# maltezfaria/LevelSetMethods.jl

Hardware: AMD Instinct MI355X
Metric: Mcells/s per RK3 step (WENO5 advect+reinit), 512^3 fp64; HBM GB/s vs peak (higher is better)
Workload: dtype f64; 1 GPU; 3D 512^3 vortex-deformation WENO5 advection + EikonalReinitializationTerm, RK3, NeumannBC, fp64; cells=134217728, integrator=RK3, arithmetic_mode=fast, parallelism=single, halo_overlap=n/a, prewarm_steps=10, exchange=n/a

## Files before the change

levelsetmethods.jl_amd/csrc/stage_brick.h:

```cpp
#pragma once
#include "stage_kernel.h"

namespace lsm {
namespace LSM_NS {

template <class LT>
struct LdsElems {
    const LT* p;
    LSM_DEV double operator[](int i) const { return (double)p[i]; }
};
template <int W, int HW, class LT>
struct BrickView {
    LdsElems<LT> T0;
    double c;
    LSM_DEV double z(int k) const { return T0[k * HW]; }
    template <int D>
    LSM_DEV double at(int k) const { return T0[k * (D == 0 ? 1 : (D == 1 ? W : HW))]; }
    template <int A, int B>
    LSM_DEV double corner(int sa, int sb) const { return T0[sa * (A == 0 ? 1 : W) + sb * (B == 1 ? W : HW)]; }
};

#ifndef LSM_BRICK_PITCH
#define LSM_BRICK_PITCH 44
#endif
struct BrickCfg {
    static constexpr int TX = 32, TY = 8, XL = 4;
    static constexpr int W = TX + 2 * XL;
    static constexpr int WP = LSM_BRICK_PITCH;
    static_assert(WP >= W && WP % 4 == 0, "rows hold the loaded elements and start on 16-byte boundaries");
};

template <int ADV, int NM, int CURV, int EIK, class ST, int AK, int NT, int BZ>
__global__ void __launch_bounds__(NT) brick_kernel(const StageArgs a, const unsigned sub_per) {
    constexpr int NDIM = 3, TX = BrickCfg::TX, TY = BrickCfg::TY, XL = BrickCfg::XL, W = BrickCfg::W, WP = BrickCfg::WP;
    constexpr int G = halo_of(ADV, NM, CURV, EIK);
    constexpr int SEG = 16 / (int)sizeof(ST), NSEG = W / SEG, PSEG = WP / SEG;
    constexpr int H = TY + 2 * G, HW = H * WP, D = BZ + 2 * G;
    constexpr int NROW = D * H, NV4 = NROW * PSEG;
    constexpr int BPT = TX * TY * BZ / NT;
    static_assert(XL >= G && XL % SEG == 0 && W % SEG == 0 && (BPT == 8 || BPT == 4) && NT % 64 == 0, "");
    __shared__ lsm_v4u vbrick[NV4];
    __shared__ unsigned short nodes[TX * TY * BZ];
    __shared__ int wsum[NT / 64];
    static_assert(2 * (sizeof(lsm_v4u) * NV4 + sizeof(unsigned short) * TX * TY * BZ + 64) <= 160 * 1024, "brick kernel: LDS budget of a gfx950 CU");
    const ST* brick = reinterpret_cast<const ST*>(vbrick);

    const unsigned nwg = a.nbrick_list * sub_per, per = (nwg + 7u) / 8u;
    const unsigned wg = (blockIdx.x % 8u) * per + blockIdx.x / 8u;
    if (blockIdx.x / 8u >= per || wg >= nwg) return;
    const unsigned tile_id = (unsigned)a.brick_list[wg / sub_per], sub = wg % sub_per;
    const unsigned tbx = tile_id % a.nb[0], tby = (tile_id / a.nb[0]) % a.nb[1], tbm = tile_id / (a.nb[0] * a.nb[1]);
    const int bx0 = tbx * TX, by0 = tby * TY;
    const int nx = a.n[0], ny = a.n[1], nm = a.n[2];
    const long long sy = a.s1, sm = a.s2;
    const int m0 = a.mb + (int)tbm * a.mc;
    const int m1 = m0 + a.mc < a.me ? m0 + a.mc : a.me;
    const int zb = m0 + (int)sub * BZ;
    if (zb >= m1) return;
    const int nz = m1 - zb < BZ ? m1 - zb : BZ;
    const int tid = threadIdx.x, lane = tid & 63, wv = tid >> 6;
    unsigned long long mbytes;
    const int mrow = tid / (TX / BPT), mq = tid % (TX / BPT), mzr = mrow / TY, myr = mrow % TY;
    {
        const unsigned char* mb_ = uniform_ptr(a.mask + (a.origin + (long long)zb * sm + (long long)by0 * sy + bx0));
        const bool rv = mzr < nz && by0 + myr < ny;
        const unsigned moff = rv ? (unsigned)mzr * (unsigned)sm + (unsigned)myr * (unsigned)sy + (unsigned)(mq * BPT) : LSM_OOB_OFFSET;
        if constexpr (BPT == 8) mbytes = __builtin_bit_cast(unsigned long long, __builtin_amdgcn_raw_buffer_load_b64(plane_rsrc(mb_), moff, 0, 0));
        else mbytes = __builtin_amdgcn_raw_buffer_load_b32(plane_rsrc(mb_), moff, 0, 0);
    }
    constexpr int RPI = NT / NSEG, NIT = (NROW + RPI - 1) / RPI, QZ = RPI / H, RY = RPI % H;
    lsm_v4u v[NIT];
    const int crow = tid / NSEG, cseg = tid - crow * NSEG;
    {
        const ST* cb = uniform_ptr(reinterpret_cast<const ST*>(a.psi) + (a.origin + (long long)(zb - G) * sm + (long long)(by0 - G) * sy + (bx0 - XL)));
        const bool cv = crow < RPI && bx0 - XL + cseg * SEG <= nx + G - 1;
        int zr = crow / H, yr = crow - zr * H;
#pragma unroll
        for (int k = 0; k < NIT; ++k) {
            int Y = by0 - G + yr, Z = zb - G + zr;
            Y = Y > ny + G - 1 ? ny + G - 1 : Y;
            Z = Z > nm + G - 1 ? nm + G - 1 : Z;
            const unsigned eo = (unsigned)(Z - (zb - G)) * (unsigned)sm + (unsigned)(Y - (by0 - G)) * (unsigned)sy + (unsigned)(cseg * SEG);
            const unsigned off = (cv && zr < D) ? (unsigned)sizeof(ST) * eo : LSM_OOB_OFFSET;
            v[k] = __builtin_bit_cast(lsm_v4u, __builtin_amdgcn_raw_buffer_load_b128(plane_rsrc(cb), off, 0, 0));
            yr += RY; zr += QZ;
            if (yr >= H) { yr -= H; ++zr; }
        }
    }
    int N;
    {
        unsigned bits = 0;
#pragma unroll
        for (int j = 0; j < BPT; ++j)
            if (((mbytes >> (8 * j)) & 0xffull) != 0 && bx0 + mq * BPT + j < nx) bits |= 1u << j;
        const int cnt = __builtin_popcount(bits);
// ... 95 lines not shown
```

levelsetmethods.jl_amd/csrc/stage_kernel.h:

```cpp
#pragma once
#include <cstdlib>
#include <type_traits>
#include "lsm_internal.h"
#include "stage_math.h"

namespace lsm {
namespace LSM_NS {

#if LSM_STRICT
constexpr bool ADV_SCALED = false;
#else
constexpr bool ADV_SCALED = true;
#endif
constexpr int adv_factor_kind(int ADV, bool PLAIN) {
#if LSM_STRICT
    return 0;
#else
    return ADV == 2 ? (LSM_T1 ? 1 : 0) | (LSM_T2 && PLAIN ? 2 : 0) : 0;
#endif
}
template <int FK>
LSM_DEV double adv_factor(const StageArgs& a, int k) {
    if constexpr (FK == 3) return a.cdt_inv_h3[k];
    else if constexpr (FK == 2) return a.cdt * a.inv_h[k];
    else if constexpr (FK == 1) return a.inv_h3[k];
    else return a.inv_h[k];
}

constexpr int halo_of(int ADV, int NM, int CURV, int EIK) {
    int g = 0;
    if (ADV == 2) g = 3;
    if (ADV == 1 && g < 1) g = 1;
    if ((NM || EIK) && g < 2) g = 2;
    if (CURV && g < 1) g = 1;
    return g;
}

template <class T>
LSM_DEV T* uniform_ptr(T* p) {
    const unsigned long long v = reinterpret_cast<unsigned long long>(p);
    const unsigned lo = __builtin_amdgcn_readfirstlane((unsigned)v), hi = __builtin_amdgcn_readfirstlane((unsigned)(v >> 32));
    return reinterpret_cast<T*>(((unsigned long long)hi << 32) | lo);
}
LSM_DEV double ld_uniform(const double* t, int i) {
    typedef const __attribute__((address_space(4))) double* cptr;
    return *((cptr)(unsigned long long)t + i);
}
typedef unsigned lsm_v2u __attribute__((ext_vector_type(2)));
LSM_DEV __amdgpu_buffer_rsrc_t plane_rsrc(const void* base, int range = (int)0x80000000u) {
    return __builtin_amdgcn_make_buffer_rsrc(const_cast<void*>(base), 0, range, 0x00020000);
}
constexpr unsigned LSM_OOB_OFFSET = 0xC0000000u;
template <class ST, int AUX = 0>
LSM_DEV double ldg(const ST* base, unsigned boff, int range = (int)0x80000000u) {
    if constexpr (sizeof(ST) == 8) return __builtin_bit_cast(double, __builtin_amdgcn_raw_buffer_load_b64(plane_rsrc(base, range), boff, 0, AUX));
    else return (double)__builtin_bit_cast(float, __builtin_amdgcn_raw_buffer_load_b32(plane_rsrc(base, range), boff, 0, AUX));
}
template <class ST, int AUX = 0>
LSM_DEV void stg(ST* base, unsigned boff, double v) {
    if constexpr (sizeof(ST) == 8) __builtin_amdgcn_raw_buffer_store_b64(__builtin_bit_cast(lsm_v2u, v), plane_rsrc(base), boff, 0, AUX);
    else __builtin_amdgcn_raw_buffer_store_b32(__builtin_bit_cast(unsigned, (float)v), plane_rsrc(base), boff, 0, AUX);
}
typedef unsigned lsm_v4u __attribute__((ext_vector_type(4)));
template <class ST, int AUX = 0>
LSM_DEV void ldg2(const ST* base, unsigned boff, double& x, double& y, int range = (int)0x80000000u) {
    if constexpr (sizeof(ST) == 8) {
        const lsm_v4u v = __builtin_bit_cast(lsm_v4u, __builtin_amdgcn_raw_buffer_load_b128(plane_rsrc(base, range), boff, 0, AUX));
        x = __builtin_bit_cast(double, lsm_v2u{v.x, v.y});
        y = __builtin_bit_cast(double, lsm_v2u{v.z, v.w});
    } else {
        const unsigned long long u = __builtin_bit_cast(unsigned long long, __builtin_amdgcn_raw_buffer_load_b64(plane_rsrc(base, range), boff, 0, AUX));
        x = (double)__builtin_bit_cast(float, (unsigned)u);
        y = (double)__builtin_bit_cast(float, (unsigned)(u >> 32));
    }
}
template <class ST, int AUX = 0>
LSM_DEV void stg2(ST* base, unsigned boff, double x, double y) {
    if constexpr (sizeof(ST) == 8) {
        const lsm_v2u a = __builtin_bit_cast(lsm_v2u, x), b = __builtin_bit_cast(lsm_v2u, y);
        __builtin_amdgcn_raw_buffer_store_b128(lsm_v4u{a.x, a.y, b.x, b.y}, plane_rsrc(base), boff, 0, AUX);
    } else {
        const unsigned long long u = (unsigned long long)__builtin_bit_cast(unsigned, (float)x) | ((unsigned long long)__builtin_bit_cast(unsigned, (float)y) << 32);
        __builtin_amdgcn_raw_buffer_store_b64(__builtin_bit_cast(lsm_v2u, u), plane_rsrc(base), boff, 0, AUX);
    }
}
LSM_DEV unsigned ldg_u8(const unsigned char* base, unsigned boff, int range) {
    return __builtin_amdgcn_raw_buffer_load_b8(
        __builtin_amdgcn_make_buffer_rsrc(const_cast<unsigned char*>(base), 0, __builtin_amdgcn_readfirstlane(range), 0x00020000), boff, 0, 0);
}

template <int NDIM, int NCOMP, bool SCALED = false, int KIND = -1, int FK = 0>
LSM_DEV void coeff_prep(const CoeffArgs& c, const StageArgs& a, int gi0, int gi1, double pre[3]) {
// ... 33 lines not shown
            const double x2 = a.lc[1] + (double)gim * a.h[1];
            out[0] = -(c.v[0] * (x2 - c.v[2]));
            if (SCALED) out[0] = out[0] * adv_factor<FK>(a, 0);
        } else {
            out[0] = pre[0];
        }
        if (NCOMP > 1) out[1] = pre[1];
        if (NCOMP > 2) out[2] = 0.0;
    } else if (kind == LSM_COEFF_SEPARABLE) {
#pragma unroll
        for (int k = 0; k < NCOMP; ++k) {
            double p = pre[k];
            if (NDIM > 1) p = p * tz[k];
            out[k] = SCALED ? p : p * c.tfac;
        }
    } else {
#pragma unroll
        for (int k = 0; k < NCOMP; ++k) {
            out[k] = ldg(uniform_ptr(c.f[k] + plane_off), ocol);
            if (SCALED) out[k] = out[k] * adv_factor<FK>(a, k);
        }
    }
}

struct PlaneTab {
    double adv[3], nm[3], curv[3];
};
template <int NDIM, int NCOMP, int KIND>
LSM_DEV void plane_tab_one(const CoeffArgs& c, const StageArgs& a, int gim, double tz[3]) {
    tz[0] = tz[1] = tz[2] = 1.0;
    if (NDIM > 1 && (KIND >= 0 ? KIND : c.kind) == LSM_COEFF_SEPARABLE) {
#pragma unroll
        for (int k = 0; k < NCOMP; ++k) tz[k] = ld_uniform(c.sep[k], (NDIM == 3 ? a.gn[0] + a.gn[1] : a.gn[0]) + gim);
    }
}
template <int NDIM, int ADV, int NM, int CURV, int AK>
LSM_DEV void plane_tab(const StageArgs& a, int gim, PlaneTab& t) {
    if constexpr (ADV != 0) plane_tab_one<NDIM, NDIM, AK>(a.adv, a, gim, t.adv);
    if constexpr (NM != 0) plane_tab_one<NDIM, 1, (AK >= 0 ? (int)LSM_COEFF_CONST : -1)>(a.nm, a, gim, t.nm);
    if constexpr (CURV != 0) plane_tab_one<NDIM, 1, (AK >= 0 ? (int)LSM_COEFF_CONST : -1)>(a.curv, a, gim, t.curv);
}

struct NodeIO {
    long long plane_off;
    unsigned ocol;
    unsigned ocold;
    int gim;
};

struct NodeOps {
    double u[3];
    double vnm;
    double bcurv;
    double s0;
    double phin;
    double out2;
    bool have_negs;
    unsigned long long negs[3];
};
template <int NDIM, int ADV, int NM, int CURV, int EIK, class ST, int AK>
LSM_DEV void node_operands(const StageArgs& a, const NodeIO& io, const double pre_adv[3], const double pre_nm[3],
                           const double pre_curv[3], const PlaneTab& pt, NodeOps& op) {
    op.u[0] = op.u[1] = op.u[2] = 0.0;
    op.vnm = op.bcurv = op.s0 = op.phin = op.out2 = 0.0;
    op.have_negs = false;
    if constexpr (ADV != 0)
        coeff_eval<NDIM, NDIM, ADV_SCALED, AK, adv_factor_kind(ADV, AK >= 0)>(a.adv, a, pre_adv, pt.adv, io.gim, io.plane_off, io.ocold, op.u);
    if constexpr (NM != 0) {
        double vv[3];
        coeff_eval<NDIM, 1, false, (AK >= 0 ? (int)LSM_COEFF_CONST : -1)>(a.nm, a, pre_nm, pt.nm, io.gim, io.plane_off, io.ocold, vv);
        op.vnm = vv[0];
    }
    if constexpr (CURV != 0) {
        double bb[3];
        coeff_eval<NDIM, 1, false, (AK >= 0 ? (int)LSM_COEFF_CONST : -1)>(a.curv, a, pre_curv, pt.curv, io.gim, io.plane_off, io.ocold, bb);
        op.bcurv = bb[0];
    }
    if constexpr (EIK == 1) op.s0 = ldg(uniform_ptr(a.s0 + io.plane_off), io.ocold);
    op.phin = ldg<ST, 0>(uniform_ptr(reinterpret_cast<const ST*>(a.phin) + io.plane_off), io.ocol,
                  __builtin_amdgcn_readfirstlane(a.base_mode == LSM_BASE_PSI ? 0 : (int)0x80000000u));
    if (AK < 0 && a.out2 && a.out2_accum) op.out2 = ldg(uniform_ptr(reinterpret_cast<const ST*>(a.out2) + io.plane_off), io.ocol);
}

template <int NDIM, int G, int W, int R = 0, int RN = 0>
struct NodeView {
    const double* T0;
    const double* Tm;
    const double* Tp;
    const double* zl;
    double c;
    LSM_DEV double z(int k) const { return zl[RN > 0 ? (R + G + k + RN) % (RN > 0 ? RN : 1) : G + k]; }
    template <int D>
    LSM_DEV double at(int k) const {
        if constexpr (D == 0) return T0[k];
        else if constexpr (D == 1 && NDIM == 3) return T0[k * W];
        else return z(k);
    }
    template <int A, int B>
    LSM_DEV double corner(int sa, int sb) const {
        if constexpr (NDIM == 3 && A == 0 && B == 1) return T0[sa + sb * W];
        else {
            const double* P = sb > 0 ? Tp : Tm;
            if constexpr (A == 0) return P[sa];
            else return P[sa * W];
        }
    }
};

#if !LSM_STRICT
LSM_DEV double sel64(int m, double x, double y) {
    return __hiloint2double((__double2hiint(x) & m) | (__double2hiint(y) & ~m), (__double2loint(x) & m) | (__double2loint(y) & ~m));
}
#ifndef LSM_NO_UNIFORM_PATHS
#define LSM_UNIFORM_PATHS 1
#else
#define LSM_UNIFORM_PATHS 0
#endif
template <int NDIM, int D, int G, int W, bool PQ, class NV>
LSM_DEV double weno_term(const NV& nv, const StageArgs& a, double v, bool have_negs, unsigned long long negs_known, double& P, double& Q) {
    const double epsf = 1.0e-99 * a.h2[D];
    auto lds = [&](auto Sc) {
        constexpr int ss = (D == 0 ? 1 : W) * decltype(Sc)::value;
        const double q0 = nv.T0[-3 * ss], q1 = nv.T0[-2 * ss], q2 = nv.T0[-ss], q4 = nv.T0[ss], q5 = nv.T0[2 * ss];
        return weno5_undivided_pq<PQ, LSM_T1 != 0>(q1 - q0, q2 - q1, nv.c - q2, q4 - nv.c, q5 - q4, epsf, P, Q);
    };
    auto reg = [&](auto Sc) {
        constexpr int ss = decltype(Sc)::value;
        return weno5_undivided_pq<PQ, LSM_T1 != 0>(nv.z(-2 * ss) - nv.z(-3 * ss), nv.z(-ss) - nv.z(-2 * ss), nv.c - nv.z(-ss),
                                      nv.z(ss) - nv.c, nv.z(2 * ss) - nv.z(ss), epsf, P, Q);
    };
    constexpr bool IN_LDS = D == 0 || (D == 1 && NDIM == 3);
    double w;
    const unsigned long long negs = have_negs ? negs_known : __builtin_amdgcn_ballot_w64(__double2hiint(v) < 0);
    if (LSM_UNIFORM_PATHS && negs == 0) {
        if constexpr (IN_LDS) w = lds(std::integral_constant<int, 1>{});
        else w = reg(std::integral_constant<int, 1>{});
    } else if (LSM_UNIFORM_PATHS && negs == __builtin_amdgcn_ballot_w64(true)) {
        if constexpr (IN_LDS) w = lds(std::integral_constant<int, -1>{});
        else w = reg(std::integral_constant<int, -1>{});
    } else {
        const int m = ~(__double2hiint(v) >> 31);
        double q[6];
        if constexpr (IN_LDS) {
            constexpr int st = D == 0 ? 1 : W;
            const int ss = (st & m) | (-st & ~m);
            q[0] = nv.T0[-3 * ss]; q[1] = nv.T0[-2 * ss]; q[2] = nv.T0[-ss];
            q[3] = nv.c;
            q[4] = nv.T0[ss]; q[5] = nv.T0[2 * ss];
        } else {
            q[0] = sel64(m, nv.z(-3), nv.z(3));
            q[1] = sel64(m, nv.z(-2), nv.z(2));
            q[2] = sel64(m, nv.z(-1), nv.z(1));
            q[3] = nv.c;
            q[4] = sel64(m, nv.z(1), nv.z(-1));
            q[5] = sel64(m, nv.z(2), nv.z(-2));
        }
        w = weno5_undivided_pq<PQ, LSM_T1 != 0>(q[1] - q[0], q[2] - q[1], q[3] - q[2], q[4] - q[3], q[5] - q[4], epsf, P, Q);
    }
    return w;
}
#endif

template <int NDIM, int D, int G, int W, class NV>
LSM_DEV double weno_dim(const NV& nv, const StageArgs& a, double v) {
    const bool up = v > 0;
    double q[6];
    if constexpr (D == 0 || (D == 1 && NDIM == 3)) {
        constexpr int st = D == 0 ? 1 : W;
        const int ss = up ? st : -st;
        q[0] = nv.T0[-3 * ss]; q[1] = nv.T0[-2 * ss]; q[2] = nv.T0[-ss];
        q[3] = nv.c;
        q[4] = nv.T0[ss]; q[5] = nv.T0[2 * ss];
    } else {
        q[0] = up ? nv.z(-3) : nv.z(3);
        q[1] = up ? nv.z(-2) : nv.z(2);
        q[2] = up ? nv.z(-1) : nv.z(1);
        q[3] = nv.c;
        q[4] = up ? nv.z(1) : nv.z(-1);
        q[5] = up ? nv.z(2) : nv.z(-2);
    }
    const double hs = up ? a.h[D] : -a.h[D];
    const double ihs = up ? a.inv_h[D] : -a.inv_h[D];
    return weno5_upwind(q, hs, ihs, 1.0e-99 * a.h2[D]);
}

template <int NDIM, int ADV, int NM, int CURV, int EIK, int G, int W, class ST, bool PLAIN, class NV>
LSM_DEV void node_update(const StageArgs& a, const NV& nv, const NodeOps& op, double& r_out, double& r_out2) {
    const double c = nv.c;
    double Ladv = 0.0, Lnm = 0.0, Lcurv = 0.0, Leik = 0.0;
#if LSM_STRICT
    constexpr bool ADV_TO_BASE = false;
#else
    constexpr bool ADV_TO_BASE = (adv_factor_kind(ADV, PLAIN) & 2) != 0;
    constexpr bool EIK_RAW = LSM_T3 && EIK == 2;
#endif
    [[maybe_unused]] double adv_base = 0.0;
    double A[3] = {0, 0, 0}, B[3] = {0, 0, 0};
#if LSM_STRICT
    constexpr bool ENO_FROM_WENO = false;
#else
    constexpr bool ENO_FROM_WENO = ADV == 2 && (NM || EIK);
#endif

    if constexpr (ADV != 0) {
        const double* u = op.u;
        auto one = [&](auto Dc) {
            constexpr int D = decltype(Dc)::value;
            const double v = u[D];
            double der;
            if constexpr (ADV == 2) {
#if LSM_STRICT
                der = weno_dim<NDIM, D, G, W>(nv, a, v);
#else
                const double w = weno_term<NDIM, D, G, W, ENO_FROM_WENO>(nv, a, v, op.have_negs, op.negs[D], A[D], B[D]);
                if constexpr (ADV_TO_BASE) {
                    adv_base = D == 0 ? -(__builtin_fabs(v) * w) : __builtin_fma(-__builtin_fabs(v), w, adv_base);
                    return 0.0;
                } else {
                    return __builtin_fabs(v) * w;
                }
#endif
            } else {
#if LSM_STRICT
                der = v > 0 ? (c - nv.template at<D>(-1)) / a.h[D] : (nv.template at<D>(1) - c) / a.h[D];
#else
                der = v > 0 ? (c - nv.template at<D>(-1)) : (nv.template at<D>(1) - c);
#endif
            }
            return v * der;
        };
        Ladv = one(std::integral_constant<int, 0>{});
        if constexpr (NDIM > 1) Ladv = Ladv + one(std::integral_constant<int, 1>{});
        if constexpr (NDIM > 2) Ladv = Ladv + one(std::integral_constant<int, 2>{});
    }

    if constexpr ((NM || EIK) && !ENO_FROM_WENO) {
        auto pr = [&](auto Dc) {
            constexpr int D = decltype(Dc)::value;
            eno2_pair(nv.template at<D>(-2), nv.template at<D>(-1), c, nv.template at<D>(1), nv.template at<D>(2), a.h[D],
                      a.h2[D], a.inv_h[D], A[D], B[D]);
// ... 160 lines not shown
            double n2 = 0.0;
            if (LSM_UNIFORM_PATHS && poss == __builtin_amdgcn_ballot_w64(true)) {
                n2 = godunov_sum<NDIM, true>(A, B, a.inv_h2, a.uniform_h != 0);
            } else if (LSM_UNIFORM_PATHS && poss == 0) {
                n2 = godunov_sum<NDIM, false>(A, B, a.inv_h2, a.uniform_h != 0);
            } else {
                const double sg = s > 0 ? 1.0 : -1.0;
#pragma unroll
                for (int d = 0; d < NDIM; ++d) n2 += godunov_term(sg, A[d], B[d], a.inv_h2[d]);
            }
            const double nrm = fast_norm(n2);
            double S;
            if constexpr (EIK == 1) {
                S = s;
            } else {
                const double d2 = __builtin_fma(n2, a.dxmin * a.dxmin, c * c);
                S = c * fast_rsqrt(__builtin_fmax(d2, 1.0e-300));
            }
            Leik = S * (nrm - 1);
        }
#endif
    }

    double base;
#if LSM_STRICT
    if (a.base_mode == LSM_BASE_PSI) base = c;
    else if (a.base_mode == LSM_BASE_RK3_S2) base = 0.75 * op.phin + 0.25 * c;
    else if (a.base_mode == LSM_BASE_RK3_S3) base = (op.phin + 2 * c) / 3;
    else base = op.phin;
#else
    __builtin_amdgcn_sched_barrier(0);
    base = __builtin_fma(a.base_a, op.phin, ADV_TO_BASE ? __builtin_fma(a.base_b, c, adv_base) : a.base_b * c);
#endif
    double b2 = !PLAIN && a.out2_accum ? op.out2 : c;
    const bool has2 = !PLAIN && a.out2 != nullptr;
    if (PLAIN || a.natural) {
        auto acc = [&](double L) {
            base -= a.cdt * L;
            if (has2) b2 -= a.cdt2 * L;
        };
        if constexpr (ADV != 0 && !ADV_TO_BASE) acc(Ladv);
        if constexpr (NM != 0) acc(Lnm);
        if constexpr (CURV != 0) acc(Lcurv);
        if constexpr (EIK != 0) acc(Leik);
    } else {
        for (int k = 0; k < a.nterms; ++k) {
            const int o = a.order[k];
            double L = Ladv;
            if (NM && o == SLOT_NM) L = Lnm;
            if (CURV && o == SLOT_CURV) L = Lcurv;
            if (EIK && o == SLOT_EIK) L = Leik;
            base -= a.cdt * L;
            b2 -= a.cdt2 * L;
        }
    }
    r_out = base;
    r_out2 = b2;
}
template <class ST, bool PLAIN>
LSM_DEV void node_store(const StageArgs& a, const NodeIO& io, bool on, double r_out, double r_out2) {
    if (!on) return;
    stg<ST, 0>(uniform_ptr(reinterpret_cast<ST*>(a.out) + io.plane_off), io.ocol, r_out);
    if (!PLAIN && a.out2) stg(uniform_ptr(reinterpret_cast<ST*>(a.out2) + io.plane_off), io.ocol, r_out2);
}

#ifndef LSM_WAVES_PER_EU
#define LSM_WAVES_PER_EU 1
#endif
#ifndef LSM_BAND_PATCH
#define LSM_BAND_PATCH 1
#endif
#ifndef LSM_ZROT
#define LSM_ZROT 1
#endif
#define LSM_BARRIER() __syncthreads()
template <int NDIM, int ADV, int NM, int CURV, int EIK, int TX, int TY, int MC, class ST, int AK, bool MASKED>
__device__ __forceinline__ void stage_tile(const StageArgs& a, unsigned tile_id, bool tail_tile, unsigned slot) {
    constexpr bool PLAIN = AK >= 0;
    constexpr bool NOMASK = PLAIN && !MASKED;
    constexpr int CK = PLAIN ? (int)LSM_COEFF_CONST : -1;
    constexpr int G = halo_of(ADV, NM, CURV, EIK);
    constexpr bool HAS_Y = NDIM == 3, MARCH = NDIM >= 2;
    constexpr int LEAD = (CURV && MARCH) ? 1 : 0;
    constexpr int NSLOT = MARCH ? 2 * LEAD + 2 : 1;
    constexpr bool ZROT = LSM_ZROT && !LSM_STRICT && NDIM == 3 && ADV == 2;
    constexpr int W = TX + 2 * G;
    constexpr int H = HAS_Y ? TY + 2 * G : 1;
    constexpr int HW = H * W;
    constexpr int NT = TX * TY;
    constexpr int NHX = 2 * G * TY;
    constexpr int WY = CURV ? W : TX;
    constexpr int NHY = HAS_Y ? 2 * G * WY : 0;
    constexpr int NH = NHX + NHY;
    constexpr int HPT = (NH + NT - 1) / NT;
    static_assert(!HAS_Y || TY > 1 || true, "");
    __shared__ double tile[NSLOT * HW];

#ifdef LSM_STAMP
    const unsigned long long st_rb = __builtin_amdgcn_s_memrealtime();
#endif
    if (a.tile_list) tile_id = (unsigned)a.tile_list[tile_id];
    else if (a.tile_active && !a.tile_active[tile_id]) return;
    const unsigned tbx = tile_id % a.nb[0], tby = (tile_id / a.nb[0]) % a.nb[1];
    const unsigned tbm = tile_id / (a.nb[0] * a.nb[1]);

    const int tid = threadIdx.x;
    int tx = tid % TX, ty = tid / TX;
    if constexpr (NDIM == 3 && TX == 32 && TY == 8 && !NOMASK) {
        if (LSM_BAND_PATCH && a.mask) { tx = 8 * (tid >> 6) + (tid & 7); ty = (tid & 63) >> 3; }
    }
    const int bx0 = tbx * TX, by0 = HAS_Y ? tby * TY : 0;
    const int gx = bx0 + tx, gy = by0 + ty;
    const int nx = a.n[0], ny = HAS_Y ? a.n[1] : 1;
    const int nm = MARCH ? a.n[NDIM - 1] : 1;
    const long long sy = HAS_Y ? a.s1 : 0;
    const long long sm = MARCH ? (NDIM == 3 ? a.s2 : a.s1) : 0;
    const bool active = gx < nx && gy < ny;
    const int cx = gx < nx ? gx : nx - 1, cy = gy < ny ? gy : ny - 1;
    const int xk0 = a.xkind[0], xk1 = a.xkind[1], yk0 = a.ykind[0], yk1 = a.ykind[1];
    const bool xmap = a.xredirect && (bx0 < G || bx0 + TX + G > nx);
    const bool ymap = HAS_Y && a.yredirect && (by0 < G || by0 + TY + G > ny);
    auto bsrc = [](int i, int n, int k0, int k1) {
        const bool left = i < 0;
        const int k = left ? -i : i - (n - 1), kind = left ? k0 : k1;
        const int per = left ? (n - 1) - k : k, ext = left ? 0 : n - 1, sym = left ? k : (n - 1) - k;
        return kind == LSM_BC_PERIODIC ? per : (kind == LSM_BC_EXTRAPOLATION ? ext : sym);
    };
    auto xsrc = [&](int i) { return (!xmap || (i >= 0 && i < nx)) ? i : bsrc(i, nx, xk0, xk1); };
    auto ysrc = [&](int i) { return (!ymap || (i >= 0 && i < ny)) ? i : bsrc(i, ny, yk0, yk1); };
    const int lxg = xsrc(gx < nx + G ? gx : nx + G - 1);
    const int lyg = HAS_Y ? ysrc(gy < ny + G ? gy : ny + G - 1) : 0;
    const long long corner = a.origin - G - (HAS_Y ? (long long)G * sy : 0);
    const unsigned ocole = (unsigned)(lxg + G) + (unsigned)(lyg + (HAS_Y ? G : 0)) * (unsigned)sy;
    const unsigned ocol = (unsigned)sizeof(ST) * ocole, ocold = 8u * ocole;
    const int mcl = a.mc > 0 ? a.mc : MC;
    const int mc = tail_tile ? a.mc_tail : mcl;
    const int m0 = MARCH ? (tail_tile ? a.mb + (int)a.nbig * mcl + (int)(tbm - a.nbig) * mc : a.mb + (int)tbm * mc) : 0;
    const int m1 = MARCH ? (m0 + mc < a.me ? m0 + mc : a.me) : 1;
    const int mlo = (MARCH && a.mredirect[0]) ? 0 : -G, mhi = (MARCH && a.mredirect[1]) ? nm - 1 : nm + G - 1;
    auto clampM = [&](int p) { return p < mlo ? mlo : (p > mhi ? mhi : p); };
    auto plane = [&](int p) { return uniform_ptr(reinterpret_cast<const ST*>(a.psi) + (corner + (long long)clampM(p) * sm)); };

    int hl[HPT > 0 ? HPT : 1];
    unsigned hg[HPT > 0 ? HPT : 1];
    bool hv[HPT > 0 ? HPT : 1];
#pragma unroll
    for (int h = 0; h < HPT; ++h) {
        const int e = tid + h * NT;
        hv[h] = e < NH;
        int lx, ly;
        if (e < NHX) {
            const int r = e % (2 * G);
            ly = e / (2 * G) + (HAS_Y ? G : 0);
            lx = r < G ? r : r + TX;
        } else {
            const int e2 = e - NHX;
            const int row = e2 / WY;
            lx = (CURV ? 0 : G) + e2 % WY;
            ly = row < G ? row : row + TY;
        }
        int X = bx0 - G + lx;
        X = xsrc(X > nx + G - 1 ? nx + G - 1 : X);
        int Y = 0;
        if (HAS_Y) {
            Y = by0 - G + ly;
            Y = ysrc(Y > ny + G - 1 ? ny + G - 1 : Y);
        }
        hl[h] = ly * W + lx;
        hg[h] = (unsigned)sizeof(ST) * ((unsigned)(X + G) + (unsigned)(Y + (HAS_Y ? G : 0)) * (unsigned)sy);
        if (!hv[h]) hg[h] = LSM_OOB_OFFSET;
    }
    const int lpos = (ty + (HAS_Y ? G : 0)) * W + tx + G;

    double pre_adv[3] = {0, 0, 0}, pre_nm[3] = {0, 0, 0}, pre_curv[3] = {0, 0, 0};
    {
        const int gi0 = cx + a.goff[0], gi1 = HAS_Y ? cy + a.goff[1] : 0;
        if constexpr (ADV != 0) coeff_prep<NDIM, NDIM, ADV_SCALED, AK, adv_factor_kind(ADV, PLAIN)>(a.adv, a, gi0, gi1, pre_adv);
        if constexpr (NM != 0) coeff_prep<NDIM, 1, false, CK>(a.nm, a, gi0, gi1, pre_nm);
        if constexpr (CURV != 0) coeff_prep<NDIM, 1, false, CK>(a.curv, a, gi0, gi1, pre_curv);
    }

    if constexpr (!MARCH) {
        const ST* P = plane(0);
        const double c = ldg(P, ocol);
        const NodeIO io{corner, ocol, ocold, 0};
        NodeOps op;
        PlaneTab pt;
        plane_tab<NDIM, ADV, NM, CURV, AK>(a, 0, pt);
        node_operands<NDIM, ADV, NM, CURV, EIK, ST, AK>(a, io, pre_adv, pre_nm, pre_curv, pt, op);
        tile[lpos] = c;
#pragma unroll
        for (int h = 0; h < HPT; ++h)
            if (hv[h]) tile[hl[h]] = ldg(P, hg[h]);
        __syncthreads();
        NodeView<NDIM, G, W> nv{tile + lpos, nullptr, nullptr, nullptr, c};
        double r1, r2;
        node_update<NDIM, ADV, NM, CURV, EIK, G, W, ST, PLAIN>(a, nv, op, r1, r2);
        node_store<ST, PLAIN>(a, io, active && (NOMASK || !a.mask || ldg_u8(uniform_ptr(a.mask + corner), ocold >> 3, (int)0x80000000u) != 0), r1, r2);
    } else {
        PlaneTab pt;
        plane_tab<NDIM, ADV, NM, CURV, AK>(a, m0 + a.goff[NDIM - 1], pt);
        double zl[2 * G + 1];
#pragma unroll
        for (int j = 0; j <= 2 * G; ++j) zl[j] = ldg(plane(m0 - G + j), ocol);
        double hp[2 * LEAD + 1][HPT > 0 ? HPT : 1];
#pragma unroll
        for (int pl = -LEAD; pl <= LEAD; ++pl) {
            const ST* P = plane(m0 + pl);
#pragma unroll
            for (int h = 0; h < HPT; ++h) hp[pl + LEAD][h] = ldg(P, hg[h]);
        }
#pragma unroll
        for (int pl = -LEAD; pl <= LEAD; ++pl) {
            const int slot = pl + LEAD;
            tile[slot * HW + lpos] = zl[G + pl];
#pragma unroll
            for (int h = 0; h < HPT; ++h)
                if (hv[h]) tile[slot * HW + hl[h]] = hp[slot][h];
        }
        const bool nomask = NOMASK || a.mask == nullptr;
        const int mrange = nomask ? 0 : (int)0x80000000u;
        long long po = corner + (long long)m0 * sm;
        unsigned mk_next = 0;
        if constexpr (!NOMASK) mk_next = ldg_u8(uniform_ptr(a.mask + po), ocold >> 3, mrange);
        const ST* Pnx = plane(m0 + G);
        const ST* Pn = plane(m0 + LEAD);
        const int plast = mhi;
        const bool any_active = __builtin_amdgcn_ballot_w64(active) != 0;
        constexpr bool SIGNS_KNOWN = PLAIN && ADV == 2 && AK != LSM_COEFF_FIELD && !LSM_STRICT;
        unsigned long long neg_pre[3] = {0, 0, 0};
        const unsigned long long all_lanes = __builtin_amdgcn_ballot_w64(true);
        if constexpr (SIGNS_KNOWN) {
#pragma unroll
            for (int d = 0; d < NDIM; ++d) neg_pre[d] = __builtin_amdgcn_ballot_w64(__double2hiint(pre_adv[d]) < 0);
        }
        __builtin_amdgcn_s_waitcnt(0x0F70);
#ifdef LSM_STAMP
        const unsigned long long st_t0 = __builtin_amdgcn_s_memtime(), st_r0 = __builtin_amdgcn_s_memrealtime();
#endif
        constexpr int ROT = ZROT ? 2 * G + 1 : 0, RM = ROT > 0 ? ROT : 1;
        auto plane_iter = [&](auto Rc, int m) {
            constexpr int R = decltype(Rc)::value;
            Pnx = uniform_ptr(m + 1 + G <= plast ? Pnx + sm : Pnx);
            Pn = uniform_ptr(m + 1 + LEAD <= plast ? Pn + sm : Pn);
            const double nxt = ldg(Pnx, ocol);
            double hn[HPT > 0 ? HPT : 1];
#pragma unroll
            for (int h = 0; h < HPT; ++h) hn[h] = ldg(Pn, hg[h]);
            const unsigned mk = mk_next;
            if constexpr (!NOMASK) mk_next = ldg_u8(uniform_ptr(a.mask + (po + sm)), ocold >> 3, mrange);
            const NodeIO io{po, ocol, ocold, m + a.goff[NDIM - 1]};
            NodeOps op;
            node_operands<NDIM, ADV, NM, CURV, EIK, ST, AK>(a, io, pre_adv, pre_nm, pre_curv, pt, op);
            if constexpr (SIGNS_KNOWN) {
                op.have_negs = true;
#pragma unroll
                for (int d = 0; d < NDIM; ++d) {
                    if (AK == LSM_COEFF_SEPARABLE) op.negs[d] = neg_pre[d] ^ (__double2hiint(pt.adv[d]) < 0 ? all_lanes : 0ull);
                    else op.negs[d] = neg_pre[d];
                }
                if (AK == LSM_COEFF_ROTATION) op.have_negs = NDIM == 3;
            }
            LSM_BARRIER();
            const bool on = active && (nomask || mk != 0);
            double r1 = 0.0, r2 = 0.0;
            if (NOMASK ? any_active : __builtin_amdgcn_ballot_w64(on) != 0) {
                const int rel = m - m0;
                const double* T0 = tile + ((rel + LEAD) % NSLOT) * HW + lpos;
                const double* Tm = tile + ((rel + LEAD + NSLOT - 1) % NSLOT) * HW + lpos;
                const double* Tp = tile + ((rel + LEAD + 1) % NSLOT) * HW + lpos;
                NodeView<NDIM, G, W, R, ROT> nv{T0, Tm, Tp, zl, zl[ROT > 0 ? (R + G) % RM : G]};
                node_update<NDIM, ADV, NM, CURV, EIK, G, W, ST, PLAIN>(a, nv, op, r1, r2);
            }
            plane_tab<NDIM, ADV, NM, CURV, AK>(a, (m + 1 < m1 ? m + 1 : m) + a.goff[NDIM - 1], pt);
            if constexpr (ROT > 0) {
                zl[R % RM] = nxt;
            } else {
#pragma unroll
                for (int j = 0; j < 2 * G; ++j) zl[j] = zl[j + 1];
                zl[2 * G] = nxt;
            }
            const int wslot = (m - m0 + 1 + 2 * LEAD) % NSLOT;
            tile[wslot * HW + lpos] = zl[ROT > 0 ? (R + 1 + G + LEAD) % RM : G + LEAD];
#pragma unroll
            for (int h = 0; h < HPT; ++h)
                if (hv[h]) tile[wslot * HW + hl[h]] = hn[h];
            node_store<ST, PLAIN>(a, io, on, r1, r2);
            po += sm;
        };
        if constexpr (ROT > 0) {
            int m = m0;
            while (m < m1) {
                bool go = true;
                auto step = [&](auto Rc) {
                    if (go) {
                        plane_iter(Rc, m);
                        ++m;
                        go = m < m1;
                    }
                };
                step(std::integral_constant<int, 0>{});
                step(std::integral_constant<int, 1>{});
                step(std::integral_constant<int, 2>{});
                if constexpr (ROT > 3) step(std::integral_constant<int, 3>{});
                if constexpr (ROT > 4) step(std::integral_constant<int, 4>{});
                if constexpr (ROT > 5) step(std::integral_constant<int, 5>{});
                if constexpr (ROT > 6) step(std::integral_constant<int, 6>{});
                if constexpr (ROT > 7) step(std::integral_constant<int, 7>{});
            }
        } else {
            for (int m = m0; m < m1; ++m) plane_iter(std::integral_constant<int, 0>{}, m);
        }
#ifdef LSM_STAMP
        if (a.stamp && threadIdx.x == 0) {
            const unsigned long long st_t1 = __builtin_amdgcn_s_memtime(), st_r1 = __builtin_amdgcn_s_memrealtime();
            a.stamp[4 * (slot % 16384u)] = st_t1 - st_t0;
            a.stamp[4 * (slot % 16384u) + 1] = st_rb;
            a.stamp[4 * (slot % 16384u) + 2] = st_r0;
            a.stamp[4 * (slot % 16384u) + 3] = st_r1;
        }
#endif
    }
}

struct TileOrder {
    unsigned ntiles, nbigt, big_per, small_per;
    __host__ __device__ explicit TileOrder(const StageArgs& a) {
        ntiles = a.tile_list ? a.ntile_list : a.nb[0] * a.nb[1] * a.nb[2];
        nbigt = a.mc_tail > 0 ? a.nb[0] * a.nb[1] * a.nbig : ntiles;
        big_per = (nbigt + 7u) / 8u;
        small_per = (ntiles - nbigt + 7u) / 8u;
    }
    __host__ __device__ unsigned per_xcd() const { return big_per + small_per; }
    __host__ __device__ bool entry(unsigned x, unsigned j, unsigned& id, bool& tail) const {
        const unsigned nb = x * big_per < nbigt ? (nbigt - x * big_per < big_per ? nbigt - x * big_per : big_per) : 0u;
        if (j < nb) { id = x * big_per + j; tail = false; return true; }
        const unsigned js = j - nb, so = nbigt + x * small_per;
        if (so + js < ntiles && js < small_per) { id = so + js; tail = true; return true; }
        return false;
    }
};

template <int NDIM, int ADV, int NM, int CURV, int EIK, int TX, int TY, int MC, class ST, int AK, bool MASKED>
__global__ void __launch_bounds__(TX* TY, (LSM_ZROT && !LSM_STRICT && NDIM == 3 && ADV == 2 && AK >= 0 && !MASKED && !CURV && !NM) ? 5 : LSM_WAVES_PER_EU)
    stage_kernel(const StageArgs a) {
    const TileOrder ord(a);
    unsigned tile_id;
    bool tail_tile;
    if (NDIM == 3 && !MASKED && a.tail_wgs && blockIdx.x >= 8u * ord.big_per) {
        __shared__ unsigned s_ticket;
        if (threadIdx.x == 0) {
            const unsigned t = __hip_atomic_fetch_add(a.tail_ctr, 1u, __ATOMIC_RELAXED, __HIP_MEMORY_SCOPE_AGENT);
            if (t + 1u == a.tail_wgs) __hip_atomic_store(a.tail_ctr, 0u, __ATOMIC_RELAXED, __HIP_MEMORY_SCOPE_AGENT);
            s_ticket = t;
        }
        __syncthreads();
        const unsigned t = (unsigned)__builtin_amdgcn_readfirstlane((int)s_ticket);
        if (t >= ord.ntiles - ord.nbigt) return;
        tile_id = ord.nbigt + t;
        tail_tile = true;
    } else if (!ord.entry(blockIdx.x % 8u, blockIdx.x / 8u, tile_id, tail_tile)) {
        return;
    }
    stage_tile<NDIM, ADV, NM, CURV, EIK, TX, TY, MC, ST, AK, MASKED>(a, tile_id, tail_tile, blockIdx.x);
}

// ... 331 lines not shown
```

levelsetmethods.jl_amd/csrc/stage_math.h:

```cpp
#pragma once
#include <hip/hip_runtime.h>

namespace lsm {
namespace LSM_NS {

#define LSM_DEV __device__ __forceinline__

LSM_DEV double positive(double x) { return x > 0.0 ? x : 0.0; }
LSM_DEV double negative(double x) { return x < 0.0 ? x : 0.0; }

#if LSM_STRICT

LSM_DEV double jl_max(double a, double b) { return (a != a || b != b) ? __builtin_nan("") : (b > a ? b : a); }

LSM_DEV double weno5_core(double v1, double v2, double v3, double v4, double v5) {
    double dphi1 = (1.0 / 3) * v1 - (7.0 / 6) * v2 + (11.0 / 6) * v3;
    double dphi2 = -(1.0 / 6) * v2 + (5.0 / 6) * v3 + (1.0 / 3) * v4;
    double dphi3 = (1.0 / 3) * v3 + (5.0 / 6) * v4 - (1.0 / 6) * v5;
    double a1 = v1 - 2 * v2 + v3, b1 = v1 - 4 * v2 + 3 * v3;
    double a2 = v2 - 2 * v3 + v4, b2 = v2 - v4;
    double a3 = v3 - 2 * v4 + v5, b3 = 3 * v3 - 4 * v4 + v5;
    double S1 = (13.0 / 12) * (a1 * a1) + (1.0 / 4) * (b1 * b1);
    double S2 = (13.0 / 12) * (a2 * a2) + (1.0 / 4) * (b2 * b2);
    double S3 = (13.0 / 12) * (a3 * a3) + (1.0 / 4) * (b3 * b3);
    double m = jl_max(jl_max(jl_max(jl_max(v1 * v1, v2 * v2), v3 * v3), v4 * v4), v5 * v5);
    double eps = 1.0e-6 * m + 1.0e-99;
    double t1 = S1 + eps, t2 = S2 + eps, t3 = S3 + eps;
    double al1 = 0.1 / (t1 * t1);
    double al2 = 0.6 / (t2 * t2);
    double al3 = 0.3 / (t3 * t3);
    double w1 = al1 / (al1 + al2 + al3);
    double w2 = al2 / (al1 + al2 + al3);
    double w3 = al3 / (al1 + al2 + al3);
    return w1 * dphi1 + w2 * dphi2 + w3 * dphi3;
}

LSM_DEV double limiter(double x, double y) {
    if (!(x * y > 0.0)) return 0.0;
    return __builtin_fabs(x) <= __builtin_fabs(y) ? x : y;
}

LSM_DEV double weno5_upwind(const double q[6], double hs, double , double ) {
    return weno5_core((q[1] - q[0]) / hs, (q[2] - q[1]) / hs, (q[3] - q[2]) / hs, (q[4] - q[3]) / hs,
                      (q[5] - q[4]) / hs);
}

LSM_DEV void eno2_pair(double m2, double m1, double c, double p1, double p2, double h, double h2, double ,
                       double& A, double& B) {
    double dm = (c - m1) / h;
    double dp = (p1 - c) / h;
    double d20 = (p1 - 2 * c + m1) / h2;
    double d2mm = (m2 - 2 * m1 + c) / h2;
    double d2pp = (c - 2 * p1 + p2) / h2;
    A = dm + 0.5 * h * limiter(d2mm, d20);
    B = dp - 0.5 * h * limiter(d2pp, d20);
}
LSM_DEV double lsm_sqrt(double x) { return __builtin_sqrt(x); }
LSM_DEV double lsm_div(double a, double b) { return a / b; }

#else

#ifndef LSM_T1
#define LSM_T1 1
#endif
#ifndef LSM_T2
#define LSM_T2 1
#endif
#ifndef LSM_T3
#define LSM_T3 1
#endif

LSM_DEV double fast_rcp(double x) {
    double r = __builtin_amdgcn_rcp(x);
    double e = __builtin_fma(-x, r, 1.0);
    return __builtin_fma(r, e, r);
}
LSM_DEV double lsm_div(double a, double b) { return a * fast_rcp(b); }

LSM_DEV double fast_rsqrt(double x) {
    double r = __builtin_amdgcn_rsq(x);
    double e = __builtin_fma(-0.5 * x * r, r, 0.5);
    return __builtin_fma(r, e, r);
}

LSM_DEV double fast_norm(double x) { return x * fast_rsqrt(__builtin_fmax(x, 1.0e-300)); }

LSM_DEV double lsm_sqrt(double x0) {
    const double x = __builtin_fmax(x0, 1.0e-300);
    double r = __builtin_amdgcn_rsq(x);
    double g = x * r, hh = 0.5 * r;
    double e = __builtin_fma(-hh, g, 0.5);
    g = __builtin_fma(g, e, g);
    hh = __builtin_fma(hh, e, hh);
    double d = __builtin_fma(-g, g, x);
    return __builtin_fma(d, hh, g);
}

LSM_DEV double minmod_fast(double x, double y);
template <bool PQ, bool X3 = false>
LSM_DEV double weno5_undivided_pq(double e1, double e2, double e3, double e4, double e5, double eps_floor, double& P, double& Q) {
    const double w1 = e2 - e1, w2 = e3 - e2, w3 = e4 - e3, w4 = e5 - e4;
    if constexpr (PQ) {
        const double hi = __builtin_fmax(w3, 0.0), lo = __builtin_fmin(w3, 0.0);
        P = __builtin_fma(0.5, __builtin_fmax(__builtin_fmin(w2, hi), lo), e3);
        Q = __builtin_fma(-0.5, __builtin_fmax(__builtin_fmin(w4, hi), lo), e4);
    }
    const double A1 = w2 - w1, A2 = w3 - w2, A3 = w4 - w3;
    const double m = __builtin_fmax(__builtin_fmax(__builtin_fmax(__builtin_fabs(e1), __builtin_fabs(e2)),
                                                   __builtin_fmax(__builtin_fabs(e3), __builtin_fabs(e4))),
                                    __builtin_fabs(e5));
    const double eps = __builtin_fma(0.75e-6 * m, m, (13.0 / 16) * __builtin_fmax(eps_floor, 1.0e-75));
    const double t2 = 0.75 * w2, t3 = 0.75 * w3;
    const double r1 = __builtin_fma(A1, A1, __builtin_fma(t2, A1 + w2, eps));
    const double r2 = __builtin_fma(A2, A2, __builtin_fma(t2, w3, eps));
    const double r3 = __builtin_fma(A3, A3, __builtin_fma(t3, w3 - A3, eps));
    const double s1 = r1 * r1, s2 = r2 * r2, s3 = r3 * r3;
    const double N = s2 * __builtin_fma(1.5, s1 * (A2 - A3), s3 * (A1 - A2));
    const double Dn = __builtin_fma(6.0, s1 * s3, s2 * __builtin_fma(3.0, s1, s3));
    if constexpr (X3) return __builtin_fma(fast_rcp(Dn), N, __builtin_fma(0.5, w2, __builtin_fma(3.0, e3, w3)));
    const double dphi2 = __builtin_fma(1.0 / 3, w3, __builtin_fma(1.0 / 6, w2, e3));
    return __builtin_fma(fast_rcp(Dn) * (1.0 / 3), N, dphi2);
}
LSM_DEV double weno5_undivided(double e1, double e2, double e3, double e4, double e5, double eps_floor) {
    double P, Q;
    return weno5_undivided_pq<false>(e1, e2, e3, e4, e5, eps_floor, P, Q);
}

LSM_DEV double weno5_upwind(const double q[6], double , double inv_hs, double eps_floor) {
    return weno5_undivided(q[1] - q[0], q[2] - q[1], q[3] - q[2], q[4] - q[3], q[5] - q[4], eps_floor) * inv_hs;
}

LSM_DEV double minmod_fast(double x, double y) {
    return __builtin_fmax(__builtin_fmin(x, y), __builtin_fmin(__builtin_fmax(x, y), 0.0));
}

LSM_DEV void eno2_pair(double m2, double m1, double c, double p1, double p2, double , double , double ,
                       double& A, double& B) {
    const double dm = c - m1, dp = p1 - c;
    const double s0 = dp - dm;
    const double smm = dm - (m1 - m2);
    const double spp = (p2 - p1) - dp;
    const double hi = __builtin_fmax(s0, 0.0), lo = __builtin_fmin(s0, 0.0);
    A = __builtin_fma(0.5, __builtin_fmax(__builtin_fmin(smm, hi), lo), dm);
    B = __builtin_fma(-0.5, __builtin_fmax(__builtin_fmin(spp, hi), lo), dp);
}
#endif

#if LSM_STRICT
LSM_DEV void godunov_sel(bool vpos, double A, double B, double& a2, double& b2) {
    double a = vpos ? positive(A) : negative(A);
    double b = vpos ? negative(B) : positive(B);
    a2 = a * a;
    b2 = b * b;
}
#else
LSM_DEV double godunov_term(double sg, double A, double B, double inv_h2) {
    const double a = __builtin_fmax(sg * A, 0.0);
    const double b = __builtin_fmin(sg * B, 0.0);
    return __builtin_fma(a, a, b * b) * inv_h2;
}
LSM_DEV double vmax0(double x) { double r; asm("v_max_f64 %0, %1, 0" : "=v"(r) : "v"(x)); return r; }
LSM_DEV double vmin0(double x) { double r; asm("v_min_f64 %0, %1, 0" : "=v"(r) : "v"(x)); return r; }
LSM_DEV double godunov_pos(double A, double B, double inv_h2) {
    const double a = vmax0(A);
    const double b = vmin0(B);
    return __builtin_fma(a, a, b * b) * inv_h2;
}
LSM_DEV double godunov_neg(double A, double B, double inv_h2) {
    const double a = vmin0(A);
    const double b = vmax0(B);
    return __builtin_fma(a, a, b * b) * inv_h2;
}
template <int NDIM, bool POS, bool RAW = false>
LSM_DEV double godunov_sum(const double* A, const double* B, const double* inv_h2, bool uniform_h) {
    if (RAW || uniform_h) {
        double s = 0.0;
#pragma unroll
        for (int d = 0; d < NDIM; ++d) {
            const double a = POS ? vmax0(A[d]) : vmin0(A[d]);
            const double b = POS ? vmin0(B[d]) : vmax0(B[d]);
            s = d == 0 ? a * a : __builtin_fma(a, a, s);
            s = __builtin_fma(b, b, s);
        }
        if constexpr (RAW) return s;
        return s * inv_h2[0];
    }
    double s = 0.0;
#pragma unroll
    for (int d = 0; d < NDIM; ++d) s += POS ? godunov_pos(A[d], B[d], inv_h2[d]) : godunov_neg(A[d], B[d], inv_h2[d]);
    return s;
}
LSM_DEV double vmax_floor(double x) { double r; asm("v_max_f64 %0, %1, %2" : "=v"(r) : "v"(x), "s"(1.0e-300)); return r; }
LSM_DEV double godunov_term_raw(double sg, double A, double B) {
// ... 16 lines not shown
```

Measured before the change: 41970 Mcells/s.

## Keep full z-stencil in LDS and store z-differences in register ring

For the plain z-rotated WENO5+reinit path, the march tile now holds 2G+1 z-planes in LDS instead of a small rotating set. The per-thread register ring stores first differences along z rather than raw values, so the z-direction WENO stencil takes ready-made differences and skips the subtractions. A precomputed max-abs helper is also added for that path. The cost is more LDS per block, which can lower occupancy, plus extra LDS writes per step.

```diff
diff --git a/levelsetmethods.jl_amd/csrc/stage_brick.h b/levelsetmethods.jl_amd/csrc/stage_brick.h
--- a/levelsetmethods.jl_amd/csrc/stage_brick.h
+++ b/levelsetmethods.jl_amd/csrc/stage_brick.h
@@ -11,6 +11,7 @@
 };
 template <int W, int HW, class LT>
 struct BrickView {
+    static constexpr bool ZD = false;
     LdsElems<LT> T0;
     double c;
     LSM_DEV double z(int k) const { return T0[k * HW]; }
diff --git a/levelsetmethods.jl_amd/csrc/stage_kernel.h b/levelsetmethods.jl_amd/csrc/stage_kernel.h
--- a/levelsetmethods.jl_amd/csrc/stage_kernel.h
+++ b/levelsetmethods.jl_amd/csrc/stage_kernel.h
@@ -8,6 +8,8 @@
 namespace LSM_NS {
 
 #if LSM_STRICT
+#define LSM_LDS7 0
+#define LSM_ZD 0
 constexpr bool ADV_SCALED = false;
 #else
 constexpr bool ADV_SCALED = true;
@@ -207,19 +209,27 @@
     if (AK < 0 && a.out2 && a.out2_accum) op.out2 = ldg(uniform_ptr(reinterpret_cast<const ST*>(a.out2) + io.plane_off), io.ocol);
 }
 
-template <int NDIM, int G, int W, int R = 0, int RN = 0>
+template <int NDIM, int G, int W, int R = 0, int RN = 0, bool ZD_ = false>
 struct NodeView {
+    static constexpr bool ZD = ZD_;
     const double* T0;
     const double* Tm;
     const double* Tp;
     const double* zl;
     double c;
-    LSM_DEV double z(int k) const { return zl[RN > 0 ? (R + G + k + RN) % (RN > 0 ? RN : 1) : G + k]; }
+    LSM_DEV double z(int k) const {
+        static_assert(!ZD_, "a ring of differences holds no march-axis values: dz()");
+        return zl[RN > 0 ? (R + G + k + RN) % (RN > 0 ? RN : 1) : G + k];
+    }
+    LSM_DEV double dz(int k) const { return zl[(R + G + k + RN) % (RN > 0 ? RN : 1)]; }
     template <int D>
     LSM_DEV double at(int k) const {
         if constexpr (D == 0) return T0[k];
         else if constexpr (D == 1 && NDIM == 3) return T0[k * W];
-        else return z(k);
+        else {
+            static_assert(!ZD_ || D < NDIM - 1, "a ring of differences holds no march-axis values");
+            return z(k);
+        }
     }
     template <int A, int B>
     LSM_DEV double corner(int sa, int sb) const {
@@ -251,8 +261,17 @@
     };
     auto reg = [&](auto Sc) {
         constexpr int ss = decltype(Sc)::value;
-        return weno5_undivided_pq<PQ, LSM_T1 != 0>(nv.z(-2 * ss) - nv.z(-3 * ss), nv.z(-ss) - nv.z(-2 * ss), nv.c - nv.z(-ss),
-                                      nv.z(ss) - nv.c, nv.z(2 * ss) - nv.z(ss), epsf, P, Q);
+        if constexpr (NV::ZD) {
+            if constexpr (ss > 0)
+                return weno5_undivided_pq<PQ, LSM_T1 != 0, true>(nv.dz(-3), nv.dz(-2), nv.dz(-1), nv.dz(0), nv.dz(1), epsf, P, Q,
+                                                                 max_abs5(nv.dz(-3), nv.dz(-2), nv.dz(-1), nv.dz(0), nv.dz(1)));
+            else
+                return weno5_undivided_pq<PQ, LSM_T1 != 0, true>(-nv.dz(2), -nv.dz(1), -nv.dz(0), -nv.dz(-1), -nv.dz(-2), epsf, P, Q,
+                                                                 max_abs5(nv.dz(2), nv.dz(1), nv.dz(0), nv.dz(-1), nv.dz(-2)));
+        } else {
+            return weno5_undivided_pq<PQ, LSM_T1 != 0>(nv.z(-2 * ss) - nv.z(-3 * ss), nv.z(-ss) - nv.z(-2 * ss), nv.c - nv.z(-ss),
+                                          nv.z(ss) - nv.c, nv.z(2 * ss) - nv.z(ss), epsf, P, Q);
+        }
     };
     constexpr bool IN_LDS = D == 0 || (D == 1 && NDIM == 3);
     double w;
@@ -265,22 +284,27 @@
         else w = reg(std::integral_constant<int, -1>{});
     } else {
         const int m = ~(__double2hiint(v) >> 31);
-        double q[6];
-        if constexpr (IN_LDS) {
-            constexpr int st = D == 0 ? 1 : W;
-            const int ss = (st & m) | (-st & ~m);
-            q[0] = nv.T0[-3 * ss]; q[1] = nv.T0[-2 * ss]; q[2] = nv.T0[-ss];
-            q[3] = nv.c;
-            q[4] = nv.T0[ss]; q[5] = nv.T0[2 * ss];
+        if constexpr (!IN_LDS && NV::ZD) {
+            w = weno5_undivided_pq<PQ, LSM_T1 != 0>(sel64(m, nv.dz(-3), -nv.dz(2)), sel64(m, nv.dz(-2), -nv.dz(1)), sel64(m, nv.dz(-1), -nv.dz(0)),
+                                                    sel64(m, nv.dz(0), -nv.dz(-1)), sel64(m, nv.dz(1), -nv.dz(-2)), epsf, P, Q);
         } else {
-            q[0] = sel64(m, nv.z(-3), nv.z(3));
-            q[1] = sel64(m, nv.z(-2), nv.z(2));
-            q[2] = sel64(m, nv.z(-1), nv.z(1));
-            q[3] = nv.c;
-            q[4] = sel64(m, nv.z(1), nv.z(-1));
-            q[5] = sel64(m, nv.z(2), nv.z(-2));
-        }
-        w = weno5_undivided_pq<PQ, LSM_T1 != 0>(q[1] - q[0], q[2] - q[1], q[3] - q[2], q[4] - q[3], q[5] - q[4], epsf, P, Q);
+            double q[6];
+            if constexpr (IN_LDS) {
+                constexpr int st = D == 0 ? 1 : W;
+                const int ss = (st & m) | (-st & ~m);
+                q[0] = nv.T0[-3 * ss]; q[1] = nv.T0[-2 * ss]; q[2] = nv.T0[-ss];
+                q[3] = nv.c;
+                q[4] = nv.T0[ss]; q[5] = nv.T0[2 * ss];
+            } else {
+                q[0] = sel64(m, nv.z(-3), nv.z(3));
+                q[1] = sel64(m, nv.z(-2), nv.z(2));
+                q[2] = sel64(m, nv.z(-1), nv.z(1));
+                q[3] = nv.c;
+                q[4] = sel64(m, nv.z(1), nv.z(-1));
+                q[5] = sel64(m, nv.z(2), nv.z(-2));
+            }
+            w = weno5_undivided_pq<PQ, LSM_T1 != 0>(q[1] - q[0], q[2] - q[1], q[3] - q[2], q[4] - q[3], q[5] - q[4], epsf, P, Q);
+        }
     }
     return w;
 }
@@ -607,11 +631,13 @@
     constexpr int G = halo_of(ADV, NM, CURV, EIK);
     constexpr bool HAS_Y = NDIM == 3, MARCH = NDIM >= 2;
     constexpr int LEAD = (CURV && MARCH) ? 1 : 0;
-    constexpr int NSLOT = MARCH ? 2 * LEAD + 2 : 1;
     constexpr bool ZROT = LSM_ZROT && !LSM_STRICT && NDIM == 3 && ADV == 2;
     constexpr int W = TX + 2 * G;
     constexpr int H = HAS_Y ? TY + 2 * G : 1;
     constexpr int HW = H * W;
+    constexpr bool LDS7 = LSM_LDS7 && ZROT && LEAD == 0 && PLAIN && !MASKED && !NM && EIK == 2 && (2 * G + 1) * HW * 8 + 64 <= 32768;
+    constexpr bool ZD = LSM_ZD && LDS7;
+    constexpr int NSLOT = LDS7 ? 2 * G + 1 : (MARCH ? 2 * LEAD + 2 : 1);
     constexpr int NT = TX * TY;
     constexpr int NHX = 2 * G * TY;
     constexpr int WY = CURV ? W : TX;
@@ -743,6 +769,14 @@
             for (int h = 0; h < HPT; ++h)
                 if (hv[h]) tile[slot * HW + hl[h]] = hp[slot][h];
         }
+        [[maybe_unused]] double zlast = 0.0;
+        if constexpr (ZD) {
+#pragma unroll
+            for (int s = 1; s <= G; ++s) tile[s * HW + lpos] = zl[G + s];
+            zlast = zl[2 * G];
+#pragma unroll
+            for (int j = 0; j < 2 * G; ++j) zl[j] = zl[j + 1] - zl[j];
+        }
         const bool nomask = NOMASK || a.mask == nullptr;
         const int mrange = nomask ? 0 : (int)0x80000000u;
         long long po = corner + (long long)m0 * sm;
@@ -791,22 +825,26 @@
             double r1 = 0.0, r2 = 0.0;
             if (NOMASK ? any_active : __builtin_amdgcn_ballot_w64(on) != 0) {
                 const int rel = m - m0;
-                const double* T0 = tile + ((rel + LEAD) % NSLOT) * HW + lpos;
+                const double* T0 = tile + (LDS7 ? R : (rel + LEAD) % NSLOT) * HW + lpos;
                 const double* Tm = tile + ((rel + LEAD + NSLOT - 1) % NSLOT) * HW + lpos;
                 const double* Tp = tile + ((rel + LEAD + 1) % NSLOT) * HW + lpos;
-                NodeView<NDIM, G, W, R, ROT> nv{T0, Tm, Tp, zl, zl[ROT > 0 ? (R + G) % RM : G]};
+                NodeView<NDIM, G, W, R, ROT, ZD> nv{T0, LDS7 ? nullptr : Tm, LDS7 ? nullptr : Tp, zl, ZD ? T0[0] : zl[ROT > 0 ? (R + G) % RM : G]};
                 node_update<NDIM, ADV, NM, CURV, EIK, G, W, ST, PLAIN>(a, nv, op, r1, r2);
             }
             plane_tab<NDIM, ADV, NM, CURV, AK>(a, (m + 1 < m1 ? m + 1 : m) + a.goff[NDIM - 1], pt);
-            if constexpr (ROT > 0) {
+            if constexpr (ZD) {
+                zl[(R + 2 * G) % RM] = nxt - zlast;
+                zlast = nxt;
+            } else if constexpr (ROT > 0) {
                 zl[R % RM] = nxt;
             } else {
 #pragma unroll
                 for (int j = 0; j < 2 * G; ++j) zl[j] = zl[j + 1];
                 zl[2 * G] = nxt;
             }
-            const int wslot = (m - m0 + 1 + 2 * LEAD) % NSLOT;
-            tile[wslot * HW + lpos] = zl[ROT > 0 ? (R + 1 + G + LEAD) % RM : G + LEAD];
+            const int wslot = LDS7 ? (R + 1) % NSLOT : (m - m0 + 1 + 2 * LEAD) % NSLOT;
+            if constexpr (ZD) tile[((R + G + 1) % NSLOT) * HW + lpos] = nxt;
+            else tile[wslot * HW + lpos] = zl[ROT > 0 ? (R + 1 + G + LEAD) % RM : G + LEAD];
 #pragma unroll
             for (int h = 0; h < HPT; ++h)
                 if (hv[h]) tile[wslot * HW + hl[h]] = hn[h];
diff --git a/levelsetmethods.jl_amd/csrc/stage_math.h b/levelsetmethods.jl_amd/csrc/stage_math.h
--- a/levelsetmethods.jl_amd/csrc/stage_math.h
+++ b/levelsetmethods.jl_amd/csrc/stage_math.h
@@ -69,6 +69,12 @@
 #ifndef LSM_T3
 #define LSM_T3 1
 #endif
+#ifndef LSM_LDS7
+#define LSM_LDS7 1
+#endif
+#ifndef LSM_ZD
+#define LSM_ZD 1
+#endif
 
 LSM_DEV double fast_rcp(double x) {
     double r = __builtin_amdgcn_rcp(x);
@@ -97,8 +103,16 @@
 }
 
 LSM_DEV double minmod_fast(double x, double y);
-template <bool PQ, bool X3 = false>
-LSM_DEV double weno5_undivided_pq(double e1, double e2, double e3, double e4, double e5, double eps_floor, double& P, double& Q) {
+LSM_DEV double max_abs5(double e1, double e2, double e3, double e4, double e5) {
+    double a, b, m;
+    asm("v_max_f64 %0, |%1|, |%2|" : "=v"(a) : "v"(e1), "v"(e2));
+    asm("v_max_f64 %0, |%1|, |%2|" : "=v"(b) : "v"(e3), "v"(e4));
+    asm("v_max_f64 %0, %1, %2" : "=v"(m) : "v"(a), "v"(b));
+    asm("v_max_f64 %0, %1, |%2|" : "=v"(m) : "v"(m), "v"(e5));
+    return m;
+}
+template <bool PQ, bool X3 = false, bool MPRE = false>
+LSM_DEV double weno5_undivided_pq(double e1, double e2, double e3, double e4, double e5, double eps_floor, double& P, double& Q, double m_pre = 0.0) {
     const double w1 = e2 - e1, w2 = e3 - e2, w3 = e4 - e3, w4 = e5 - e4;
     if constexpr (PQ) {
         const double hi = __builtin_fmax(w3, 0.0), lo = __builtin_fmin(w3, 0.0);
@@ -106,9 +120,10 @@
         Q = __builtin_fma(-0.5, __builtin_fmax(__builtin_fmin(w4, hi), lo), e4);
     }
     const double A1 = w2 - w1, A2 = w3 - w2, A3 = w4 - w3;
-    const double m = __builtin_fmax(__builtin_fmax(__builtin_fmax(__builtin_fabs(e1), __builtin_fabs(e2)),
-                                                   __builtin_fmax(__builtin_fabs(e3), __builtin_fabs(e4))),
-                                    __builtin_fabs(e5));
+    const double m = MPRE ? m_pre
+                          : __builtin_fmax(__builtin_fmax(__builtin_fmax(__builtin_fabs(e1), __builtin_fabs(e2)),
+                                                          __builtin_fmax(__builtin_fabs(e3), __builtin_fabs(e4))),
+                                           __builtin_fabs(e5));
     const double eps = __builtin_fma(0.75e-6 * m, m, (13.0 / 16) * __builtin_fmax(eps_floor, 1.0e-75));
     const double t2 = 0.75 * w2, t3 = 0.75 * w3;
     const double r1 = __builtin_fma(A1, A1, __builtin_fma(t2, A1 + w2, eps));
```

New measurement: 42870 Mcells/s (median of 6 runs). 2.1% higher.
